# ArchieGertsman/spark-sched-sim

Measured on AMD Instinct MI355X. Metric: env-steps/sec at 4096 batched envs (TPC-H, 10 exec), higher is better.
Workload: dtype int64+f64

## Files before the change

__graft_entry__.py:

```python
from __future__ import annotations

import os.path as osp
import subprocess
import sys

ROOT = osp.dirname(osp.abspath(__file__))
if ROOT not in sys.path:
    sys.path.insert(0, ROOT)


def build() -> None:
    from spark_sched_sim_amd import build as hip_build

    from concurrent.futures import ThreadPoolExecutor

    sys.path.insert(0, osp.join(ROOT, "tests"))
    from gpu_variant import build_variant

    with ThreadPoolExecutor(2) as pool:
        variant = pool.submit(build_variant, "vecforms")
        out = hip_build.build(verbose=True)
        variant.result()
    assert osp.exists(out)
    subprocess.run(["make", "-s", "-C", osp.join(ROOT, "oracle")], check=True)
    import ctypes

    import spark_sched_sim_amd
    from spark_sched_sim_amd.binding import EXPORTS

    lib = ctypes.CDLL(out)
    for sym in EXPORTS:
        getattr(lib, sym)
    print("build ok:", out)


def smoke() -> None:
    import numpy as np
    import torch

    sys.path.insert(0, osp.join(ROOT, "tests"))
    from oracle_binding import OracleEnv
    from spark_sched_sim_amd import VecSparkSchedSimEnv, workload
    from spark_sched_sim_amd.digest import splitmix64

    assert torch.cuda.is_available(), "smoke() needs a GPU"
    cfg = dict(num_executors=5, job_arrival_cap=8, job_arrival_rate=1.0e-4, moving_delay=1500.0, warmup_delay=500.0)
    pack = workload.default_pack()
    B, T = 8, 60
    env = VecSparkSchedSimEnv(cfg, B, device="cuda:0", pack=pack)
    env.reset(seed=1000)
    oracles = [OracleEnv(pack, cfg) for _ in range(B)]
    for k, o in enumerate(oracles):
        assert o.reset(1000 + k) == 0
    done = [False] * B
    for t in range(T):
        oi = env.obs_i32.cpu().numpy()
        of = env.obs_f64.cpu().numpy()
        nodes = env.nodes.cpu().numpy()
        si = np.full(B, -1, np.int32)
        ne = np.ones(B, np.int32)
        for k, o in enumerate(oracles):
            if done[k]:
                continue
            info, onodes, _, _, _ = o.obs()
            assert (int(oi[k, 0]), int(oi[k, 3]), int(oi[k, 4]), int(oi[k, 5])) == (info.n_nodes, info.n_schedulable, info.num_committable_execs, info.source_job_idx), (t, k)
            assert np.float64(of[k, 1]).view(np.uint64) == np.float64(info.wall_time).view(np.uint64), (t, k)
            assert np.array_equal(nodes[k, : info.n_nodes].view(np.uint32), onodes.view(np.uint32)), (t, k)
            h = splitmix64(((1000 + k) << 32) ^ t)
            si[k] = h % info.n_schedulable if info.n_schedulable else -1
            ne[k] = 1 + splitmix64(h) % max(1, info.num_committable_execs)
        env.step({"stage_idx": torch.from_numpy(si).cuda(), "num_exec": torch.from_numpy(ne).cuda()})
        rew = env.obs_f64[:, 0].cpu().numpy()
        for k, o in enumerate(oracles):
            if done[k]:
                continue
            e, r, term = o.step(int(si[k]), int(ne[k]))
            assert e == 0 and np.float64(r).view(np.uint64) == np.float64(rew[k]).view(np.uint64), (t, k, e)
            done[k] = term
    env.close()
    print("smoke ok")


if __name__ == "__main__":
    build()
    if "--smoke" in sys.argv:
        smoke()
```

spark_sched_sim_amd/csrc/sss_sim.h:

```cpp
#pragma once
#ifdef SSS_WIDE
#ifdef SSS_TIMELINE
#define SSS_KNAME(name) name##_wide_tl
#else
#define SSS_KNAME(name) name##_wide
#endif
#else
#ifdef SSS_TIMELINE
#define SSS_KNAME(name) name##_tl
#else
#define SSS_KNAME(name) name
#endif
#endif
#include "../../include/sss.h"
#include "sss_layout.h"
#include <wave_rt.h>


struct alignas(16) SssScratch {
  uint8_t pool8[8];
  uint8_t pool8b[8];
  uint64_t rng_buf[64];
  int32_t rng_pos, pad0_[3];
  uint8_t setA[SSS_SET_TABLE];
// ... 349 lines not shown
  int cap = dynamic_partition ? (g_c.E + denom - 1) / denom : g_c.E;
  int src_rank = -1, first_rank = -1, first_sup = 0;
  uint32_t base = 0;
  int n_chunks = (A + 63) / 64;
  if (n_chunks == 0) n_chunks = 1;
  for (int ch = 0; ch < n_chunks; ch++) {
    int k = ch * 64 + lane;
    bool valid = k < A;
    int j = valid ? (int)lds_active()[k] : 0;
    uint64_t sm = 0, act = 0;
    int sup = 0, gs = 0;
    if (valid) {
      const SssJob& job = (*jobp(j));
      sm = job.sched_mask, act = job.active_mask, sup = job.supply, gs = job.gs_base;
    }
    int best = find_stage_dev(sm, act, gs);
    uint32_t cnt = (uint32_t)popc64(sm);
    uint32_t excl = wave_scan_excl_u32(cnt);
    uint32_t total = wave_sum_u32(cnt);
    uint32_t abs_rank = base + excl + (best >= 0 ? (uint32_t)popc64(sm & (bit64(best) - 1)) : 0u);
    bool is_src = valid && j == src_job;
    uint64_t m_src = wave_ballot(is_src && best >= 0);
    uint64_t m_el = wave_ballot(valid && best >= 0 && !(sup >= cap || is_src));
    if (m_src != 0 && src_rank < 0) src_rank = (int)wave_bcast_u32(abs_rank, ctz64(m_src));
    if (m_el != 0 && first_rank < 0) {
      int l = ctz64(m_el);
      first_rank = (int)wave_bcast_u32(abs_rank, l);
      first_sup = (int)wave_bcast_u32((uint32_t)sup, l);
    }
    base += total;
  }
  if (src_rank >= 0) {
    stage_idx = src_rank, num_exec = ncommit;
  } else if (first_rank >= 0) {
    int room = cap - first_sup;
    stage_idx = first_rank, num_exec = ncommit < room ? ncommit : room;
  } else {
    stage_idx = -1, num_exec = ncommit;
  }
  if (num_exec < 1) num_exec = 1;
}


SSS_DEV double stage_work(const JobView& v, int s) { return (double)(float)v.st[s].remaining * (double)v.dur[s]; }

SSS_DEV double job_work(const JobView& v, uint64_t act) {
  double w = 0.0;
  for (uint64_t m = act; m; m &= m - 1) w += stage_work(v, ctz64(m));
  return w;
}

SSS_DEV double wfair_weight(double W, int alpha) {
  if (alpha == 0) return 1.0;
  const double x = W > 1.0 ? W : 1.0;
  const int k = alpha < 0 ? -alpha : alpha;
  double p = x;
  for (int i = 1; i < k; i++) p *= x;
  return alpha > 0 ? p : 1.0 / p;
}

SSS_DEV void policy_wfair(int alpha, int& stage_idx, int& num_exec) {
  int lane = wave_lane();
  int A = g_hot.h.n_active;
  uint32_t srck = g_hot.h.curr_source;
  int ncommit = obs_num_committable();
  int src_job = (srck == POOL_NONE || srck == POOL_COMMON) ? -1 : key_job(srck);
  const int E = g_c.E;
  int n_chunks = (A + 63) / 64;
  if (n_chunks == 0) n_chunks = 1;
  double S = 0.0, w_last = 1.0;
  for (int ch = 0; ch < n_chunks; ch++) {
    int k = ch * 64 + lane;
    double w = 1.0;
    if (k < A) {
      const JobView v = jobview(lds_active()[k]);
      w = wfair_weight(job_work(v, v.job->active_mask), alpha);
    }
    int n = A - ch * 64 < 64 ? A - ch * 64 : 64;
    for (int l = 0; l < n; l++) S += wave_readlane_f64(w, l);
    w_last = w;
  }
  int src_rank = -1, first_rank = -1, first_sup = 0, first_cap = 0;
  uint32_t base = 0;
  for (int ch = 0; ch < n_chunks; ch++) {
    int k = ch * 64 + lane;
    bool valid = k < A;
    int j = valid ? (int)lds_active()[k] : 0;
    uint64_t sm = 0, act = 0;
    int sup = 0, gs = 0, cap = 0;
    if (valid) {
      const JobView v = jobview(j);
      sm = v.job->sched_mask, act = v.job->active_mask, sup = v.job->supply, gs = v.job->gs_base;
      const double w = n_chunks == 1 ? w_last : wfair_weight(job_work(v, act), alpha);
      const double c = __builtin_ceil(((double)E * w) / S);
      cap = c < 1.0 ? 1 : (c > (double)E ? E : (int)c);
    }
    int best = find_stage_dev(sm, act, gs);
    uint32_t cnt = (uint32_t)popc64(sm);
    uint32_t excl = wave_scan_excl_u32(cnt);
    uint32_t total = wave_sum_u32(cnt);
    uint32_t abs_rank = base + excl + (best >= 0 ? (uint32_t)popc64(sm & (bit64(best) - 1)) : 0u);
    bool is_src = valid && j == src_job;
    uint64_t m_src = wave_ballot(is_src && best >= 0);
    uint64_t m_el = wave_ballot(valid && best >= 0 && !(sup >= cap || is_src));
    if (m_src != 0 && src_rank < 0) src_rank = (int)wave_bcast_u32(abs_rank, ctz64(m_src));
    if (m_el != 0 && first_rank < 0) {
      int l = ctz64(m_el);
      first_rank = (int)wave_bcast_u32(abs_rank, l);
      first_sup = (int)wave_bcast_u32((uint32_t)sup, l);
      first_cap = (int)wave_bcast_u32((uint32_t)cap, l);
    }
    base += total;
  }
  if (src_rank >= 0) {
    stage_idx = src_rank, num_exec = ncommit;
  } else if (first_rank >= 0) {
    int room = first_cap - first_sup;
    stage_idx = first_rank, num_exec = ncommit < room ? ncommit : room;
  } else {
    stage_idx = -1, num_exec = ncommit;
  }
  if (num_exec < 1) num_exec = 1;
}

SSS_DEV void policy_sjfcp(int& stage_idx, int& num_exec) {
  int lane = wave_lane();
  int A = g_hot.h.n_active;
  int ncommit = obs_num_committable();
  int n_chunks = (A + 63) / 64;
  if (n_chunks == 0) n_chunks = 1;
  uint64_t best_key = ~0ull;
  int best_j = -1;
  uint32_t best_base = 0, base = 0;
  for (int ch = 0; ch < n_chunks; ch++) {
    int k = ch * 64 + lane;
    bool valid = k < A;
    int j = valid ? (int)lds_active()[k] : 0;
    uint64_t sm = 0;
    double W = 0.0;
    if (valid) {
      const JobView v = jobview(j);
      sm = v.job->sched_mask;
      W = job_work(v, v.job->active_mask);
    }
    uint32_t cnt = (uint32_t)popc64(sm);
    uint32_t excl = wave_scan_excl_u32(cnt);
    uint32_t total = wave_sum_u32(cnt);
    bool cand = valid && sm != 0;
    uint64_t key = cand ? f64_bits(W) : ~0ull;
    uint64_t mn = wave_min_u64(key);
    uint64_t hit = wave_ballot(cand && key == mn);
    if (hit != 0 && mn < best_key) {
      int l = ctz64(hit);
      best_key = mn, best_j = (int)wave_bcast_u32((uint32_t)j, l), best_base = base + wave_bcast_u32(excl, l);
    }
    base += total;
  }
  stage_idx = -1, num_exec = ncommit;
  if (best_j >= 0) {
    const JobView v = jobview(best_j);
    const uint64_t act = v.job->active_mask, sm = v.job->sched_mask;
    const bool mine = (act >> lane) & 1;
    const double w = mine ? stage_work(v, lane) : 0.0;
    const uint64_t kids = mine ? g_c.pk.stage_child_mask[v.job->gs_base + lane] & act : 0;
    double cp = w;
    for (int r = 0; r <= 64; r++) {
      double mx = 0.0;
      uint64_t rem = kids;
      while (wave_ballot(rem != 0)) {
        const bool take = rem != 0;
        const int c = take ? ctz64(rem) : lane;
        rem &= rem - 1;
        const double vc = wave_bcast_f64(cp, c);
        if (take && vc > mx) mx = vc;
      }
      const double nc = kids ? w + mx : w;
      const bool changed = wave_ballot(f64_bits(nc) != f64_bits(cp)) != 0;
      cp = nc;
      if (!changed) break;
    }
    const bool cand = (sm >> lane) & 1;
    const uint64_t key = cand ? ~f64_bits(cp) : ~0ull;
    const uint64_t mn = wave_min_u64(key);
    const uint64_t hit = wave_ballot(cand && key == mn);
    if (hit != 0) stage_idx = (int)best_base + popc64(sm & (bit64(ctz64(hit)) - 1));
  }
  if (num_exec < 1) num_exec = 1;
}

SSS_DEV uint64_t splitmix64(uint64_t x) {
  x += 0x9E3779B97F4A7C15ull;
  uint64_t z = x;
  z = (z ^ (z >> 30)) * 0xBF58476D1CE4E5B9ull;
  z = (z ^ (z >> 27)) * 0x94D049BB133111EBull;
  return z ^ (z >> 31);
}

SSS_DEV void policy_hash(int p_none_permille, int& stage_idx, int& num_exec) {
  uint64_t seed = g_hot.h.seed;
  uint64_t step = (uint64_t)g_hot.h.ep_steps;
  int n_sched = g_hot.h.n_sched;
  int ncommit = obs_num_committable();
  wave_sync();
  uint64_t h = splitmix64((seed << 32) ^ step), h2 = splitmix64(h), h3 = splitmix64(h2);
  if (n_sched == 0 || (int)(h3 % 1000) < p_none_permille)
    stage_idx = -1;
  else
    stage_idx = (int)(h % (uint64_t)n_sched);
  num_exec = 1 + (int)(h2 % (uint64_t)(ncommit > 0 ? ncommit : 1));
}

enum { SSS_POLICY_FAIR = 0, SSS_POLICY_FIFO = 1, SSS_POLICY_HASH = 2, SSS_POLICY_WFAIR = 3, SSS_POLICY_SJFCP = 4 };

template <bool kHeuristics = true>
SSS_DEV void run_policy(int policy, int param, int& stage_idx, int& num_exec) {
  PROF3(29);
  if (policy == SSS_POLICY_HASH)
    policy_hash(param, stage_idx, num_exec);
  else if (kHeuristics && policy == SSS_POLICY_WFAIR)
    policy_wfair(param, stage_idx, num_exec);
  else if (kHeuristics && policy == SSS_POLICY_SJFCP)
    policy_sjfcp(stage_idx, num_exec);
  else
    policy_fair(policy == SSS_POLICY_FAIR, stage_idx, num_exec);
}

#ifndef SSS_TIMELINE
SSS_KERNEL void SSS_KNAME(sss_policy_kernel)(SssKernelArgs a, int policy, int param, int32_t* stage_idx, int32_t* num_exec) {
  int env = wave_env();
  uint8_t* base = (uint8_t*)a.B.state + (size_t)env * a.L.env_stride;
  ctx_init();
  env_begin_readonly(base);
  int si, ne;
  run_policy(policy, param, si, ne);
  if (wave_lane() == 0) stage_idx[env] = si, num_exec[env] = ne;
}
#endif

#define ROLLOUT_BODY(kHeuristics) \
  int env = wave_env(); \
  uint8_t* base = (uint8_t*)a.B.state + (size_t)env * a.L.env_stride; \
  ctx_init(); \
  env_begin(base); \
  for (int it = 0; it < n_steps; it++) { \
    bool over = wave_ballot(g_hot.h.terminated || g_hot.h.need_reset) != 0; \
    double reward = 0.0; \
    if (over) { \
      if (!auto_reset || wave_ballot(g_hot.h.err != 0) != 0) break;  \
      do_reset(a.L, g_hot.h.seed + seed_stride, g_hot.h.time_limit); \
    } else { \
      int si, ne; \
      run_policy<kHeuristics>(policy, param, si, ne); \
      reward = do_step<true>(si, ne); \
    } \
    write_observation(a.L, a.B, env, reward); \
    wave_sync(); \
  } \
  env_end(base); \
  prof3_flush();

#ifdef __HIP__
#define SSS_ROLLOUT_HEURISTICS false
#else
#define SSS_ROLLOUT_HEURISTICS true
#endif
SSS_KERNEL void SSS_KNAME(sss_rollout_kernel)(SssKernelArgs a, int policy, int param, int n_steps, int auto_reset, uint64_t seed_stride) {
  ROLLOUT_BODY(SSS_ROLLOUT_HEURISTICS)
}
#ifdef __HIP__
SSS_KERNEL void SSS_KNAME(sss_rollout_heur_kernel)(SssKernelArgs a, int policy, int param, int n_steps, int auto_reset, uint64_t seed_stride) {
  ROLLOUT_BODY(true)
}
#endif
#undef ROLLOUT_BODY
#undef SSS_ROLLOUT_HEURISTICS

#undef H
#undef FAIL
#undef CHECK
```

spark_sched_sim_amd/csrc/sss_sim_env.h:

```cpp
#undef SSS_SRC_ID
#define SSS_SRC_ID 11
SSS_DEV void env_begin(const uint8_t* base) {
  PROF3(23);
  int lane = wave_lane();
  {
    const SssHot* g = (const SssHot*)base;
    if (lane < (int)(sizeof(SssHdr) / 16)) ((uint4*)&g_hot.h)[lane] = ((const uint4*)&g->h)[lane];
    for (int x = lane; x < SSS_MAX_EXEC; x += 64) {
      SssEvSlot ev;
      ev.t = __builtin_inf(), ev.seq = 0, ev.info = EV_NONE;
      uint32_t loc = POOL_NONE, csrc = 0, cdst = 0, cseq = 0;
      int16_t job = -1, cn = 0;
      int8_t ts = -1;
      uint8_t exe = 0;
      if (x < g_c.E)
        ev = g->ev[x], loc = g->ex_loc[x], job = g->ex_job[x], ts = g->ex_task_stage[x], exe = g->ex_executing[x], csrc = g->c_src[x],
        cdst = g->c_dst[x], cseq = g->c_seq[x], cn = g->c_n[x];
      g_hot.ev[x] = ev, g_hot.ex_loc[x] = loc, g_hot.ex_job[x] = job, g_hot.ex_task_stage[x] = ts, g_hot.ex_executing[x] = exe;
      g_hot.c_src[x] = csrc, g_hot.c_dst[x] = cdst, g_hot.c_seq[x] = cseq, g_hot.c_n[x] = cn;
    }
  }
  for (int i = lane; i < g_c.J_cap; i += 64) lds_slot_of()[i] = SLOT_NONE;
  for (int x = lane; x < g_c.E; x += 64) lds_exdesc()[x].gs = -1;
  lds_slot_ref()[lane] = 0;
// ... 224 lines not shown
  uint32_t not_max = 0xFFFFFFFFu;
  for (int k = lane; k < n_old + n_act; k += 64) {
    const uint32_t id = k < n_old ? lds_old_active()[k] : lds_active()[k - n_old];
    tab[id] = (uint16_t)(id + 2);
    not_max = ~id < not_max ? ~id : not_max;
  }
  wave_sync();
  uint32_t cnt = 0;
  for (int i = lane * 8; i < cap; i += 64 * 8) {
    const uint4 q = *(const uint4*)(tab + i);
    const uint32_t w[4] = {q.x, q.y, q.z, q.w};
    for (int b = 0; b < 4; b++) cnt += ((w[b] & 0xFFFFu) != 0 ? 1u : 0u) + ((w[b] >> 16) != 0 ? 1u : 0u);
  }
  const uint32_t n = wave_sum_u32(cnt);
  const uint32_t max_id = n ? ~wave_min_u32(not_max) : 0u;
  const uint32_t mask = n < 5 ? 7u : (n < 19 ? 31u : (n < 77 ? 127u : (n < 307 ? 511u : 2047u)));
  if (max_id <= mask && (int)mask < cap) {
    if (lane == 0) g_sc.jobset_mask = (int32_t)mask;
  } else {
    wave_sync();
    if (lane == 0) jobtime_build_set();
  }
  wave_sync();
}

SSS_DEV double jobtime_sum() {
  PROF3(25);
  int lane = wave_lane();
  double wall_old = g_sc.wall_old, wall = g_hot.h.wall_time;
  int mask = g_sc.jobset_mask;
  double beta = g_c.P.beta;
  const uint16_t* tab = lds_jobset();
  double job_time = 0.0;
  for (int b0 = 0; b0 <= mask; b0 += 256) {
    double ta[4], tc[4];
    bool live[4];
    SSS_UNROLL4 for (int u = 0; u < 4; u++) {
      const int b = b0 + 64 * u;
      const uint32_t en = (b + lane) <= mask ? (uint32_t)tab[b + lane] : 0u;
      live[u] = en >= 2;
      ta[u] = 0.0, tc[u] = 0.0;
      if (live[u]) ta[u] = g_c.t_arrival[(int)en - 2], tc[u] = g_c.t_completed[(int)en - 2];
    }
    SSS_UNROLL4 for (int u = 0; u < 4; u++) {
      if (b0 + 64 * u > mask) break;
      double term = 0.0;
      if (live[u]) {
        double start = ta[u] > wall_old ? ta[u] : wall_old;
        double end = tc[u] < wall ? tc[u] : wall;
        if (beta == 0.0)
          term = end - start;
        else
          term = fd_exp(-beta * 1e-3 * (start - wall_old)) - fd_exp(-beta * 1e-3 * (end - wall_old));
      }
      uint64_t m = wave_ballot(live[u]);
      while (m) {
        int k = ctz64(m);
        m &= m - 1;
        job_time += wave_bcast_f64(term, k);
      }
    }
  }
  if (beta > 0.0) job_time /= beta;
  return job_time;
}


SSS_DEV int handle_popped(const FastCtx& f, int ex, double t_win, uint32_t info_win, uint64_t& t_slow) {
  UTRACE("handle_popped");
  PROF3(31);
  if (ex == POP_EMPTY) return 1;
  H.n_events++;
  g_sc.events_this_step++;
  int fast = 0;
  if (ex >= 0 && info_kind(info_win) == EV_TASK_FINISHED)
    fast = fast_task_completion(f, ex, t_win, info_job(info_win), info_stage(info_win), info_slot(info_win));
  if (fast > 0) {
    H.n_fast++;
    if (H.curr_source == POOL_NONE) return 0;
  } else {
    if (fast < 0) FAIL(SSS_ERR_NO_DURATION);
    uint64_t ts0 = wave_clock();
    if (fast < 0) {
    } else if (ex == POP_ARRIVAL) {
      int job = H.next_arrival;
      H.wall_time = H.next_arrival_t;
      H.next_arrival++;
      H.next_arrival_t = H.next_arrival < H.J ? g_c.t_arrival[H.next_arrival] : __builtin_inf();
      handle_job_arrival(job);
    } else {
      SssHot& hot = g_hot;
      SssEvSlot sl = hot.ev[ex];
      H.wall_time = sl.t;
      hot.ev[ex].t = __builtin_inf();
      hot.ev[ex].info = EV_NONE;
      if (info_slot(sl.info) != INFO_SLOT_NONE) lds_slot_ref()[info_slot(sl.info)]--;
      g_sc.pinned_job = info_job(sl.info);
      if (info_kind(sl.info) == EV_TASK_FINISHED) {
        STAT(43, 1), STAT(44, H.curr_source != POOL_NONE), STAT(45, info_slot(sl.info) == INFO_SLOT_NONE);
        handle_task_completion(ex, info_job(sl.info), info_stage(sl.info));
      }
      else {
        STAT(39, 1), STAT(40, H.curr_source != POOL_NONE), STAT(41, info_slot(sl.info) == INFO_SLOT_NONE);
        STAT(42, (*stgp(info_job(sl.info), info_stage(sl.info))).remaining == 0);
        handle_executor_arrival(ex, info_job(sl.info), info_stage(sl.info));
      }
      g_sc.pinned_job = -1;
    }
    if (g_sc.pending_free >= 0) {
      int k = lds_slot_of()[g_sc.pending_free];
      if (k != SLOT_NONE && lds_slot_ref()[k] == 0) cache_release(g_sc.pending_free);
      g_sc.pending_free = -1;
    }
    t_slow += wave_clock() - ts0;
  }
  if (H.err) return 1;
  if (trk_num_committable() > 0) {
    publish_scan_inputs();
    return 2;
  }
  return 0;
}

template <bool FUSED = false>
SSS_DEV bool resume_simulation(int budget = 0) {
  PROF3(26);
  int lane = wave_lane();
  FastCtx f;
  fastctx_load(f);
  const int rng_need = 2 * (f.E < 20 ? f.E : 20);
  (void)rng_need;
  for (;;) {
    uint64_t t_slow = 0;
    int status;
    do {
      status = 0;
      double t_win = 0.0;
      uint32_t info_win = 0;
      wave_sync();
      if (budget > 0 && g_sc.events_this_step - g_sc.events_at_launch >= budget) return true;
      double next_arrival_t = g_hot.h.next_arrival < g_hot.h.J ? g_hot.h.next_arrival_t : __builtin_inf();
      int ex = pop_event_wave(next_arrival_t, t_win, info_win);
      const bool head_cached = ex >= 0 && info_slot(info_win) != INFO_SLOT_NONE;
      if (head_cached || (ex >= 0 && info_kind(info_win) == EV_TASK_FINISHED)) {
        int handled = 0;
        const bool tf = info_kind(info_win) == EV_TASK_FINISHED;
        const bool tasks_left = tf && head_cached && f.cstages[info_slot(info_win) * f.SP + info_stage(info_win)].remaining > 0;
        if (!head_cached) {
          handled = fast_run<FUSED>(f);
        } else if (tasks_left) {
          handled = fast_run<FUSED>(f);
        } else {
#ifndef SSS_NO_BATCH
          if (64 - g_sc.rng_pos < rng_need) {
            rng_refill();
          }
#endif
          handled = tf ? batch_released_events(f, ex) : batch_arrival_events(f, ex);
#ifndef SSS_NO_LEAN
          if (handled == 0) handled = tf ? lean_released(f, ex, t_win, info_win) : lean_arrival(f, ex, t_win, info_win);
#endif
          if (handled == 0 && tf) preflush_completing_job(f, info_win, t_win);
        }
        if (handled > 0) continue;
      }
      if (lane == 0) status = handle_popped(f, ex, t_win, info_win, t_slow);
      status = (int)wave_lane0_u32((uint32_t)status);
    } while (status == 0);
    if (lane == 0) {
      g_sc.f_done = status == 1, g_sc.f_scan = status == 2;
      H.prof[0] += t_slow;
    }
    wave_sync();
    if (g_sc.f_done) {
      if (lane == 0) {
        for (int a = 0; a < H.n_active; a++) (*jobp(lds_active()[a])).sched_mask = 0;
        H.n_sched = 0;
      }
      wave_sync();
      return false;
    }
    int n = find_schedulable_all();
    if (n > 0) {
      if (lane == 0) H.n_sched = n;
      wave_sync();
      return false;
    }
    publish_idle_mask();
    if (lane == 0) {
      move_idle_executors_all(POOL_NONE);
      H.curr_source = POOL_NONE;
      g_sc.idle_valid = 0;
    }
    wave_sync();
  }
}

SSS_DEV void do_reset(const SssLayout& L, uint64_t seed, double time_limit) {
  PROF3(27);
  int lane = wave_lane();
  SssHot& hot = g_hot;
  for (int i = lane; i < g_c.J_cap; i += 64) lds_slot_of()[i] = SLOT_NONE;
  lds_slot_ref()[lane] = 0;
  wave_sync();
  if (lane == 0) {
    g_sc.free_slots = g_c.P.n_slots >= 64 ? ~0ull : (bit64(g_c.P.n_slots) - 1);
    g_sc.pending_free = -1, g_sc.pinned_job = -1, g_sc.idle_valid = 0, g_sc.fi_detach = 0;
    uint64_t n_steps = H.n_steps, n_events = H.n_events, model_bytes = H.model_bytes;
    int dur_head = H.dur_head, dur_n = H.dur_n, episodes = H.episodes, last_ep_steps = H.last_ep_steps;
    double last_ep_return = H.last_ep_return, last_ep_wall = H.last_ep_wall;
    uint64_t prof[5];
    for (int i = 0; i < 5; i++) prof[i] = H.prof[i];
    uint64_t n_fast_keep = H.n_fast, n_batched_keep = H.n_batched, n_rounds_keep = H.n_rounds, pad0_keep = H.err_line;
    SssHdr z = {};
    H = z;
    for (int i = 0; i < 5; i++) H.prof[i] = prof[i];
    H.n_fast = n_fast_keep, H.n_batched = n_batched_keep, H.n_rounds = n_rounds_keep, H.err_line = pad0_keep;
    H.n_steps = n_steps, H.n_events = n_events, H.model_bytes = model_bytes;
    H.dur_head = dur_head, H.dur_n = dur_n, H.episodes = episodes;
    H.last_ep_steps = last_ep_steps, H.last_ep_return = last_ep_return, H.last_ep_wall = last_ep_wall;
    H.seed = seed, H.time_limit = time_limit;
    H.graph_version = 1;
    H.curr_source = POOL_COMMON;
    g_sc.events_this_step = 0;
    g_sc.reset_more = 0;
    if (!(time_limit < __builtin_inf()) && g_c.P.cap_cfg <= 0) {
      H.err = SSS_ERR_NO_LIMIT;
      H.need_reset = 1;
    } else {
      rng_seed(H, seed);
      g_sc.rng_pos = 64;
      H.J = 0;
      g_sc.reset_t = 0.0, g_sc.reset_more = 1;
    }
  }
  wave_sync();
  while (g_sc.reset_more) {
    rng_refill();
    if (lane == 0) {
      double t = g_sc.reset_t;
      int J = H.J;
      bool more = true;
      while (g_sc.rng_pos <= 56) {
        if (!(t < time_limit && (g_c.P.cap_cfg <= 0 || J < g_c.P.cap_cfg))) {
          more = false;
          break;
        }
        if (J >= g_c.J_cap) {
          H.err = SSS_ERR_CAPACITY;
          H.need_reset = 1;
          more = false;
          break;
        }
        int q = (int)rng_integers((uint32_t)g_c.pk.n_queries);
        int size = (int)rng_integers((uint32_t)g_c.pk.n_sizes);
        (*jobp(J)).gs_base = q * g_c.pk.n_sizes + size;
        g_c.t_arrival[J] = t;
        J++;
        t += g_c.P.mean_interarrival * rng_standard_exponential();
      }
      H.J = J, g_sc.reset_t = t, g_sc.reset_more = more ? 1 : 0;
    }
    wave_sync();
  }
  for (int x = lane; x < SSS_MAX_EXEC; x += 64) {
    hot.ev[x].t = __builtin_inf(), hot.ev[x].seq = 0, hot.ev[x].info = EV_NONE;
    hot.ex_loc[x] = x < g_c.E ? POOL_COMMON : POOL_NONE;
    hot.ex_job[x] = -1;
    hot.ex_task_stage[x] = -1, hot.ex_executing[x] = 0;
    hot.c_src[x] = POOL_NONE, hot.c_dst[x] = POOL_NONE, hot.c_seq[x] = 0, hot.c_n[x] = 0;
    if (x < g_c.E) tl_reset_row(x);
  }
  wave_sync();
  int J = hot.h.J;
  for (int j = lane; j < J; j += 64) {
    SssJob& job = (*jobp(j));
    int tmpl = job.gs_base;
    int gs = g_c.pk.tmpl_stage_off[tmpl];
    int ns = g_c.pk.tmpl_stage_off[tmpl + 1] - gs;
    uint64_t frontier = 0;
    for (int s = 0; s < ns; s++)
      if (g_c.pk.stage_parent_mask[gs + s] == 0) frontier |= bit64(s);
    job.active_mask = ns >= 64 ? ~0ull : (bit64(ns) - 1);
    job.frontier_mask = frontier;
    job.selected_mask = 0, job.sched_mask = 0, job.sat_mask = 0, job.local_mask = 0;
    job.supply = 0, job.sat_count = 0, job.completion_order = -1;
    job.n_stages = (uint8_t)ns;
    job.n_edges = (uint8_t)(g_c.pk.tmpl_edge_off[tmpl + 1] - g_c.pk.tmpl_edge_off[tmpl]);
    job.edge_off = g_c.pk.tmpl_edge_off[tmpl];
    job.gs_base = gs;
    g_c.t_completed[j] = __builtin_inf();
  }
  wave_sync();
  for (int i = lane; i < J * g_c.SP; i += 64) {
    int j = i / g_c.SP, s = i - j * g_c.SP;
    const SssJob& job = (*jobp(j));
    SssStage st = {0, 0, 0, 0};
    float d = 0.0f;
    if (s < (int)job.n_stages) {
      st.remaining = g_c.pk.stage_num_tasks[job.gs_base + s];
      d = (float)g_c.pk.stage_rough[job.gs_base + s];
    }
    g_c.stages[i] = st;
    g_c.durations[i] = d;
  }
  int n_pools = 1 + g_c.J_cap + J * g_c.SP;
  for (int p = lane; p < n_pools; p += 64) {
    *(uint4*)(g_c.pool_hdr + p) = p == 0 ? ((const uint4*)g_c.pk.common_pool)[0] : mk_u4(7u, 0u, 0u, 0u);
  }
  {
    const uint32_t cmask = ((const uint32_t*)g_c.pk.common_pool)[0] & 0xFFFFu;
    if (cmask != 7)
      for (uint32_t w = (uint32_t)lane; w < (cmask + 1) / 16; w += 64) ((uint4*)g_c.pool_tab)[w] = ((const uint4*)g_c.pk.common_pool)[1 + w];
// ... 141 lines not shown
```

spark_sched_sim_amd/csrc/sss_sim_lean.h:

```cpp
#undef SSS_SRC_ID
#define SSS_SRC_ID 9
SSS_DEV int lean_released(const FastCtx& f, int ex, double t_ev, uint32_t info) {
  UTRACE("lean_released");
#ifdef SSS_NO_BATCH
  return 0;
#endif
  PROF3(32);
  const int lane = wave_lane();
  const uint32_t slot = info_slot(info);
  const int s = info_stage(info), j = info_job(info);
  const SssStage st_old = f.cstages[slot * f.SP + s];
  const uint32_t source = g_hot.h.curr_source;
  const int n_commits = g_hot.h.n_commits;
  const int A = g_hot.h.n_active;
  const uint32_t counter0 = g_hot.h.counter;
  uint32_t h0 = g_hot.h.rng_has32, u32_0 = g_hot.h.rng_u32;
  const uint32_t sp = key_stage_pool(j, s);
  const bool mine = st_old.remaining == 0 && st_old.executing >= 2 && g_hot.ex_job[ex] == j && pair_staging_fits(f.E);
  const CommitHit hit = commit_first_wave(sp, false, mine, n_commits);
  STAT(120, 1), STAT(121, hit.ci < 0);
  if (hit.ci < 0) return 0;
  const int ci = hit.ci;
  const uint32_t dst = hit.dst;
  const int c_left = hit.num - 1;
// ... 27 lines not shown
              const uint64_t m = ready_mask_of_job(*q, true);
              if (m) ss = ctz64_nz(m);
            }
          }
        }
        const uint64_t hm = wave_ballot(ss >= 0);
        if (hm) tj = (int)wave_readlane_u32((uint32_t)jj, ctz64_nz(hm)), ts = (int)wave_readlane_u32((uint32_t)ss, ctz64_nz(hm));
      }
    }
  }
  int type;
  uint32_t tslot = slot;
  SssStage st_t = {0, 0, 0, 0};
  if (tj < 0)
    type = job_sat ? RL_IDLE_COMMON : RL_IDLE_JOB;
  else {
    if (tj != j) tslot = f.slot_of[tj];
    if (tslot == SLOT_NONE) {
      ok = false, type = RL_SEND;
    } else {
      st_t = f.cstages[tslot * f.SP + ts];
      ok = ok && st_t.remaining > 0;
      type = tj != j ? RL_SEND : ((jp->frontier_mask & bit64(ts)) ? RL_START : RL_PARK);
    }
  }
  const uint32_t enters = type == RL_START ? key_stage_pool(j, ts) : (type == RL_SEND ? POOL_NONE : (type == RL_IDLE_COMMON ? POOL_COMMON : key_job_pool(j)));
  ok = ok && (source == POOL_NONE || enters != source);
  const PoolPairRegs pr = pool_pair_fetch(sp, enters, enters != POOL_NONE);
  const bool start = ok && type == RL_START;
  int n_local = 0, li = 0, ri = 0;
  int4 da = mk_i4(0, 0, 0, 0), db = da;
  if (start) {
    n_local = local_count(jp->local_mask);
    ok = n_local > 0 && n_local <= f.E && ts != s;
    if (ok) {
      executor_interval(n_local, li, ri);
      const int gs2 = jp->gs_base + ts;
      da = *(const int4*)eff_row(f.eff, gs2, li, 2);
      db = li != ri ? *(const int4*)eff_row(f.eff, gs2, ri, 2) : da;
      ok = (da.y & LENW_LEN) > 1 && (db.y & LENW_LEN) > 1;
    }
  }
  const bool refill = start && ok && g_sc.rng_pos > 62;
  STAT(122, !ok);
  if (wave_ballot(!ok) != 0) return 0;
  if (refill) rng_refill();
  int pos = g_sc.rng_pos;
  double dur = 0.0;
  bool reject = false;
  if (start) {
    int4 dd = da;
    if (li != ri) {
      const double left = (double)exec_level_value(li), right = (double)exec_level_value(ri);
      const int rand_pt = 1 + (int)(u64_to_unit(g_sc.rng_buf[pos]) * (right - left));
      pos += 1;
      if (!((double)rand_pt <= (double)n_local - left)) dd = db;
    }
    uint32_t u32;
    if (h0)
      u32 = u32_0, h0 = 0;
    else {
      const uint64_t x = g_sc.rng_buf[pos];
      pos += 1;
      u32 = (uint32_t)x, u32_0 = (uint32_t)(x >> 32), h0 = 1;
    }
    const uint32_t len = (uint32_t)(dd.y & LENW_LEN);
    const uint64_t mm = (uint64_t)u32 * len;
    reject = (uint32_t)mm < len;
    dur = (double)f.durations[dd.x + (int)(mm >> 32)];
    if (dd.y >> 30) dur += g_c.P.warmup_delay;
  }
  if (wave_ballot(reject) != 0) return 0;
  STAT(111, 1), STAT(112 + type, 1), STAT(117, backup);
  PairImg so, sn;
  pool_pair_stage(pr, enters != POOL_NONE, so, sn);
  {
    bool was = pair_remove(so, (uint32_t)ex);
    CHECK(was);
    so.s.aux -= 1;
    if (enters != POOL_NONE) pair_add(sn, (uint32_t)ex);
    wave_sync();
    pool_pair_flush_one(sp, so);
    if (enters != POOL_NONE) pool_pair_flush_one(enters, sn);
  }
  if (lane == 0) {
    SssHdr& h = g_hot.h;
    h.wall_time = t_ev;
    h.n_events += 1, h.n_batched += 1, h.n_rounds += 1;
    g_sc.events_this_step += 1;
    f.cstages[slot * f.SP + s].executing = (int16_t)(st_old.executing - 1);
    g_hot.c_n[ci] = (int16_t)c_left;
    if (c_left == 0) {
      const int last = h.n_commits - 1;
      g_hot.c_src[ci] = g_hot.c_src[last], g_hot.c_dst[ci] = g_hot.c_dst[last], g_hot.c_n[ci] = g_hot.c_n[last], g_hot.c_seq[ci] = g_hot.c_seq[last];
      h.n_commits = last;
    }
    if (dst == POOL_COMMON) {
      h.supply_none -= 1;
      CHECK(h.supply_none >= 0);
    } else {
      const JobView v = jobview(j2);
      const int c = (int)v.st[s2].commit_to - 1;
      CHECK(c >= 0);
      v.st[s2].commit_to = (uint8_t)c;
      update_sat(v, s2);
      if (j2 != j) v.job->supply = (int16_t)(v.job->supply - 1);
    }
    uint32_t new_info = EV_NONE;
    double new_t = __builtin_inf();
    if (tj >= 0) {
      SssStage* spt = f.cstages + tslot * f.SP + ts;
      SssJob* jpt = f.cjobs + tslot;
      SssStage t2 = *spt;
      if (type == RL_START) {
        t2.remaining = t2.remaining - 1, t2.executing = (int16_t)(t2.executing + 1);
        if (t2.remaining == 0) jpt->sat_count = (int16_t)(jpt->sat_count + 1);
        f.cdur[slot * f.SP + ts] = (float)dur;
        new_t = t_ev + dur, new_info = ev_info(EV_TASK_FINISHED, j, ts, slot);
        g_sc.rng_pos = pos, h.rng_has32 = h0, h.rng_u32 = u32_0;
      } else if (type == RL_SEND) {
        t2.moving_to = (uint8_t)(t2.moving_to + 1);
        jpt->supply = (int16_t)(jpt->supply + 1);
        jp->supply = (int16_t)(jp->supply - 1);
        new_t = t_ev + g_c.P.moving_delay, new_info = ev_info(EV_EXECUTOR_READY, tj, ts, tslot);
      }
      *spt = t2;
      const int demand = (int)t2.remaining - ((int)t2.moving_to + (int)t2.commit_to);
      const uint64_t m = jpt->sat_mask;
      jpt->sat_mask = demand <= 0 ? (m | bit64(ts)) : (m & ~bit64(ts));
    }
    g_hot.ex_executing[ex] = type == RL_START ? 1 : 0;
    g_hot.ex_loc[ex] = enters;
    if (type == RL_START) g_hot.ex_task_stage[ex] = (int8_t)ts;
    if (type == RL_PARK) g_hot.ex_task_stage[ex] = -1;
    if (type == RL_SEND || type == RL_IDLE_COMMON) {
      jp->local_mask = local_without(jp->local_mask, ex);
      g_hot.ex_job[ex] = -1, g_hot.ex_task_stage[ex] = -1;
      if (type == RL_IDLE_COMMON) tl_append(ex, t_ev, -1);
    }
    SssEvSlot sl;
    sl.t = new_t, sl.seq = counter0, sl.info = new_info;
    if (new_info == EV_NONE) sl.seq = g_hot.ev[ex].seq;
    g_hot.ev[ex] = sl;
    if (new_info != EV_NONE) h.counter = counter0 + 1;
    if (type != RL_START) {
      lds_slot_ref()[slot]--;
      if (type == RL_SEND) lds_slot_ref()[tslot]++;
    }
  }
  wave_sync();
  return 1;
}

SSS_DEV int lean_arrival(const FastCtx& f, int ex, double t_ev, uint32_t info) {
  UTRACE("lean_arrival");
#ifdef SSS_NO_BATCH
  return 0;
#endif
  PROF3(38);
  const int lane = wave_lane();
  const uint32_t slot = info_slot(info);
  const int s = info_stage(info), j = info_job(info);
  SssJob* const jp = f.cjobs + slot;
  SssStage* const stp = f.cstages + slot * f.SP + s;
  const SssStage st = *stp;
  const uint32_t source = g_hot.h.curr_source;
  const uint32_t counter0 = g_hot.h.counter;
  uint32_t h0 = g_hot.h.rng_has32, u32_0 = g_hot.h.rng_u32;
  const uint64_t local = jp->local_mask;
  const bool start = (jp->frontier_mask & bit64(s)) != 0;
  const uint32_t jkey = key_job_pool(j), skey = key_stage_pool(j, s);
  const PoolPairRegs pr = pool_pair_fetch(jkey, skey, start);
  bool ok = pair_staging_fits(f.E) && st.remaining > 0 && st.moving_to > 0 && g_hot.ex_task_stage[ex] < 0 && (source == POOL_NONE || source != (start ? skey : jkey));
  const int n_local = local_count(local) + 1;
  int li = 0, ri = 0;
  int4 da = mk_i4(0, 0, 0, 0), db = da;
  if (ok && start) {
    ok = n_local <= f.E;
    if (ok) {
      executor_interval(n_local, li, ri);
      const int gs = jp->gs_base + s;
      da = *(const int4*)eff_row(f.eff, gs, li, 0);
      db = li != ri ? *(const int4*)eff_row(f.eff, gs, ri, 0) : da;
      ok = (da.y & LENW_LEN) > 1 && (db.y & LENW_LEN) > 1;
    }
  }
  const bool refill = ok && start && g_sc.rng_pos > 62;
  if (wave_ballot(!ok) != 0) return 0;
  if (refill) rng_refill();
  int pos = g_sc.rng_pos;
  double dur = 0.0;
  bool reject = false;
  if (start) {
    int4 dd = da;
    if (li != ri) {
      const double left = (double)exec_level_value(li), right = (double)exec_level_value(ri);
      const int rand_pt = 1 + (int)(u64_to_unit(g_sc.rng_buf[pos]) * (right - left));
      pos += 1;
      if (!((double)rand_pt <= (double)n_local - left)) dd = db;
    }
    uint32_t u32;
    if (h0)
      u32 = u32_0, h0 = 0;
    else {
      const uint64_t x = g_sc.rng_buf[pos];
      pos += 1;
      u32 = (uint32_t)x, u32_0 = (uint32_t)(x >> 32), h0 = 1;
    }
    const uint32_t len = (uint32_t)(dd.y & LENW_LEN);
    const uint64_t mm = (uint64_t)u32 * len;
    reject = (uint32_t)mm < len;
    dur = (double)f.durations[dd.x + (int)(mm >> 32)];
    if (dd.y >> 30) dur += g_c.P.warmup_delay;
  }
  if (wave_ballot(reject) != 0) return 0;
  STAT(125, 1), STAT(126, start);
  PairImg sj, ss;
  pool_pair_stage(pr, start, sj, ss);
  {
    pair_add(sj, (uint32_t)ex);
    bool was = pair_remove(sj, (uint32_t)ex);
    CHECK(was);
    if (start) pair_add(ss, (uint32_t)ex); else pair_add(sj, (uint32_t)ex);
    wave_sync();
    pool_pair_flush_one(jkey, sj);
    if (start) pool_pair_flush_one(skey, ss);
  }
  if (lane == 0) {
    SssHdr& h = g_hot.h;
    h.wall_time = t_ev;
    h.n_events += 1, h.n_batched += 1, h.n_rounds += 1;
    g_sc.events_this_step += 1;
    jp->local_mask = local_with(local, ex);
    g_hot.ex_job[ex] = (int16_t)j;
    tl_append(ex, t_ev, j);
    SssStage t2 = st;
    t2.moving_to = (uint8_t)(t2.moving_to - 1);
    SssEvSlot sl = g_hot.ev[ex];
    if (start) {
      t2.remaining = t2.remaining - 1, t2.executing = (int16_t)(t2.executing + 1);
      if (t2.remaining == 0) jp->sat_count = (int16_t)(jp->sat_count + 1);
      f.cdur[slot * f.SP + s] = (float)dur;
      sl.t = t_ev + dur, sl.seq = counter0, sl.info = ev_info(EV_TASK_FINISHED, j, s, slot);
      h.counter = counter0 + 1;
      g_sc.rng_pos = pos, h.rng_has32 = h0, h.rng_u32 = u32_0;
      g_hot.ex_task_stage[ex] = (int8_t)s, g_hot.ex_executing[ex] = 1, g_hot.ex_loc[ex] = skey;
    } else {
      sl.t = __builtin_inf(), sl.info = EV_NONE;
      g_hot.ex_task_stage[ex] = -1, g_hot.ex_loc[ex] = jkey;
      lds_slot_ref()[slot]--;
    }
    g_hot.ev[ex] = sl;
    *stp = t2;
    const int demand = (int)t2.remaining - ((int)t2.moving_to + (int)t2.commit_to);
    const uint64_t m = jp->sat_mask;
    jp->sat_mask = demand <= 0 ? (m | bit64(s)) : (m & ~bit64(s));
  }
  wave_sync();
  return 1;
}

SSS_DEV void preflush_completing_job(const FastCtx& f, uint32_t info, double t_ev) {
#ifdef SSS_NO_BATCH
  return;
#endif
  const int lane = wave_lane();
  const uint32_t slot = info_slot(info);
  const int s = info_stage(info), j = info_job(info);
  const SssStage st = f.cstages[slot * f.SP + s];
  const SssJob* jp = f.cjobs + slot;
  const bool completes = st.remaining == 0 && st.executing == 1 && jp->active_mask == bit64(s) && (int)jp->sat_count == (int)jp->n_stages && pair_staging_fits(f.E);
  if (wave_ballot(completes) == 0) return;
  PROF3(40);
  const uint32_t jkey = key_job_pool(j);
  if (lane == 0) {
    int m = 0;
    if (pool_size(jkey) > 0) {
      SetImg<uint8_t> idle = get_idle_source_executors(jkey);
      for (uint32_t i = 0; i <= idle.mask; i++)
        if (idle.tab[i] >= 2) g_sc.fi_e[m++] = (uint8_t)(idle.tab[i] - 2);
    }
    g_sc.fi_m = m;
  }
  wave_sync();
  const int m = g_sc.fi_m;
  if (m == 0) return;
  const PoolPairRegs pr = pool_pair_fetch(jkey, POOL_COMMON, true);
  PairImg so, sn;
  pool_pair_stage(pr, true, so, sn);
  LocalGroup moved = local_group();
  pair_remove_many(so, g_sc.fi_e, 0, m);
  for (int i = 0; i < m; i++) {
    const uint32_t e = g_sc.fi_e[i];
    local_group_add(moved, (int)e);
    pair_add(sn, e);
  }
  wave_sync();
  pool_pair_flush_one(jkey, so);
  pool_pair_flush_one(POOL_COMMON, sn);
  if (lane == 0) {
    SssJob* jw = f.cjobs + slot;
    local_group_detach(jw, moved);
    for (int i = 0; i < m; i++) {
      const int e = g_sc.fi_e[i];
      g_hot.ex_loc[e] = POOL_COMMON, g_hot.ex_job[e] = -1, g_hot.ex_task_stage[e] = -1;
      tl_append(e, t_ev, -1);
// ... 6 lines not shown
```

Before: 24.07 million.

## Add lean source-release fast path for last-task completions without commitments

Adds a lean_source_release device path that, when a task finishes on a stage with no pending commitment, updates stage/job masks, the executor pool pair and the header in one wave pass instead of falling through to the slow single-lane handle_popped path. It also skips the batch/lean attempts when the stage's last executing task finishes, since those can't apply there. It swaps a broadcast helper for readlane and builds a no-batch variant alongside the main build. The trade-off is more code divergence and extra commit lookups on the task-finished path, plus correctness risk in the hand-written state updates.

Measured after the change: 23.36 million. -2.9%, worse.

```diff
diff --git a/__graft_entry__.py b/__graft_entry__.py
--- a/__graft_entry__.py
+++ b/__graft_entry__.py
@@ -17,10 +17,13 @@
     sys.path.insert(0, osp.join(ROOT, "tests"))
     from gpu_variant import build_variant
 
-    with ThreadPoolExecutor(2) as pool:
+    from source_release_util import build_nobatch
+
+    with ThreadPoolExecutor(3) as pool:
         variant = pool.submit(build_variant, "vecforms")
+        nobatch = pool.submit(build_nobatch)
         out = hip_build.build(verbose=True)
-        variant.result()
+        variant.result(), nobatch.result()
     assert osp.exists(out)
     subprocess.run(["make", "-s", "-C", osp.join(ROOT, "oracle")], check=True)
     import ctypes
diff --git a/spark_sched_sim_amd/csrc/sss_sim.h b/spark_sched_sim_amd/csrc/sss_sim.h
--- a/spark_sched_sim_amd/csrc/sss_sim.h
+++ b/spark_sched_sim_amd/csrc/sss_sim.h
@@ -525,7 +525,7 @@
     uint64_t hit = wave_ballot(cand && key == mn);
     if (hit != 0 && mn < best_key) {
       int l = ctz64(hit);
-      best_key = mn, best_j = (int)wave_bcast_u32((uint32_t)j, l), best_base = base + wave_bcast_u32(excl, l);
+      best_key = mn, best_j = (int)wave_readlane_u32((uint32_t)j, l), best_base = base + wave_readlane_u32(excl, l);
     }
     base += total;
   }
diff --git a/spark_sched_sim_amd/csrc/sss_sim_env.h b/spark_sched_sim_amd/csrc/sss_sim_env.h
--- a/spark_sched_sim_amd/csrc/sss_sim_env.h
+++ b/spark_sched_sim_amd/csrc/sss_sim_env.h
@@ -400,13 +400,30 @@
           handled = fast_run<FUSED>(f);
         } else {
 #ifndef SSS_NO_BATCH
-          if (64 - g_sc.rng_pos < rng_need) {
-            rng_refill();
+          const bool last_task = !FUSED && tf && f.cstages[info_slot(info_win) * f.SP + info_stage(info_win)].executing < 2;
+#else
+          const bool last_task = false;
+#endif
+          if (!last_task) {
+#ifndef SSS_NO_BATCH
+            if (64 - g_sc.rng_pos < rng_need) {
+              rng_refill();
+            }
+#endif
+            handled = tf ? batch_released_events(f, ex) : batch_arrival_events(f, ex);
+#ifndef SSS_NO_LEAN
+            if (handled == 0) handled = tf ? lean_released(f, ex, t_win, info_win) : lean_arrival(f, ex, t_win, info_win);
+#endif
           }
-#endif
-          handled = tf ? batch_released_events(f, ex) : batch_arrival_events(f, ex);
-#ifndef SSS_NO_LEAN
-          if (handled == 0) handled = tf ? lean_released(f, ex, t_win, info_win) : lean_arrival(f, ex, t_win, info_win);
+#if !defined(SSS_NO_BATCH) && !defined(SSS_NO_LEAN)
+          if (!FUSED && tf && handled == 0) {
+            const CommitHit hit = commit_first_wave(key_stage_pool(info_job(info_win), info_stage(info_win)), false, true, g_hot.h.n_commits);
+            const int released = hit.ci < 0 ? lean_source_release(f, ex, t_win, info_win) : 0;
+            if (released > 0) {
+              status = released == 2 ? 2 : 0;
+              continue;
+            }
+          }
 #endif
           if (handled == 0 && tf) preflush_completing_job(f, info_win, t_win);
         }
diff --git a/spark_sched_sim_amd/csrc/sss_sim_lean.h b/spark_sched_sim_amd/csrc/sss_sim_lean.h
--- a/spark_sched_sim_amd/csrc/sss_sim_lean.h
+++ b/spark_sched_sim_amd/csrc/sss_sim_lean.h
@@ -203,6 +203,77 @@
   return 1;
 }
 
+SSS_DEV int lean_source_release(const FastCtx& f, int ex, double t_ev, uint32_t info) {
+  UTRACE("lean_source_release");
+#ifdef SSS_NO_BATCH
+  return 0;
+#endif
+  PROF3(41);
+  const int lane = wave_lane();
+  const uint32_t slot = info_slot(info);
+  const int s = info_stage(info), j = info_job(info);
+  const SssStage st_old = f.cstages[slot * f.SP + s];
+  SssJob* const jp = f.cjobs + slot;
+  const uint64_t active = jp->active_mask, frontier = jp->frontier_mask;
+  const int n_stages = jp->n_stages, gs_base = jp->gs_base;
+  const bool job_sat = (int)jp->sat_count == n_stages;
+  const uint32_t sp = key_stage_pool(j, s), jkey = key_job_pool(j);
+  const bool mine = st_old.remaining == 0 && st_old.executing >= 1 && g_hot.ex_job[ex] == j && g_hot.ex_loc[ex] == sp && (active & bit64(s)) != 0 && (frontier & bit64(s)) != 0;
+  const bool completes = st_old.executing == 1;
+  const uint64_t active2 = active & ~bit64(s);
+  const PoolPairRegs pr = pool_pair_fetch(sp, jkey, true);
+  const bool my_stage = completes && lane < n_stages && ((active2 >> lane) & 1ull) != 0;
+  uint64_t children = 0, parents = 0;
+  if (completes) children = g_c.pk.stage_child_mask[gs_base + s];
+  if (my_stage) parents = g_c.pk.stage_parent_mask[gs_base + lane];
+  const uint64_t all = n_stages >= 64 ? ~0ull : (bit64(n_stages) - 1);
+  const uint64_t completed = all & ~active2;
+  const uint64_t newm = wave_ballot(my_stage && ((children >> lane) & 1ull) != 0 && (parents & ~completed) == 0);
+  const bool moves = newm != 0;
+  const bool empties = completes && active2 == 0;
+  STAT(71, 1), STAT(75, !mine), STAT(76, mine && empties), STAT(77, mine && !empties && !pair_staging_fits(f.E)), STAT(78, mine && !empties && pair_staging_fits(f.E) && moves && job_sat);
+  const bool ok = mine && !empties && pair_staging_fits(f.E) && !(moves && job_sat);
+  if (wave_ballot(!ok) != 0) return 0;
+  STAT(72, !completes), STAT(73, completes && !moves), STAT(74, moves);
+  int n_committable;
+  if (moves) {
+    PairImg so, sn;
+    pool_pair_stage(pr, true, so, sn);
+    bool was = pair_remove(so, (uint32_t)ex);
+    CHECK(was);
+    pair_add(sn, (uint32_t)ex);
+    wave_sync();
+    pool_pair_flush_one(sp, so);
+    pool_pair_flush_one(jkey, sn);
+    n_committable = (int)sn.s.used - (int)sn.s.aux;
+    STAT(85, sn.mask_before != 7 || sn.s.mask != 7), STAT(86, so.mask_before != 7);
+  } else
+    n_committable = (int)(pr.rec_a.y & 0xFFFFu) - (int)(pr.rec_a.y >> 16);
+  CHECK(n_committable >= 0);
+  STAT(79, n_committable > 0);
+  if (lane == 0) {
+    SssHdr& h = g_hot.h;
+    h.wall_time = t_ev;
+    h.n_events += 1, h.n_batched += 1, h.n_rounds += 1;
+    g_sc.events_this_step += 1;
+    f.cstages[slot * f.SP + s].executing = (int16_t)(st_old.executing - 1);
+    if (completes) {
+      jp->active_mask = active2;
+      jp->frontier_mask = (frontier & ~bit64(s)) | newm;
+      h.graph_version++;
+    }
+    g_hot.ex_executing[ex] = 0;
+    g_hot.ex_task_stage[ex] = -1;
+    if (moves) g_hot.ex_loc[ex] = jkey;
+    h.curr_source = moves ? jkey : sp;
+    g_hot.ev[ex].t = __builtin_inf(), g_hot.ev[ex].info = EV_NONE;
+    lds_slot_ref()[slot]--;
+    if (n_committable > 0) g_sc.m_n_active = h.n_active, g_sc.m_src_job = j;
+  }
+  wave_sync();
+  return n_committable > 0 ? 2 : 1;
+}
+
 SSS_DEV int lean_arrival(const FastCtx& f, int ex, double t_ev, uint32_t info) {
   UTRACE("lean_arrival");
 #ifdef SSS_NO_BATCH
```
